# hellojialee/Improved-Body-Parts

Measured on NVIDIA H100. Metric: grouping images/sec @128x128 heatmaps, 30 persons/img, higher is better.
Workload: dtype f32 body-part maps, f32 keypoint maps; f64 coordinates/scores

## Files before the change

### improved_body_parts_b200/csrc/common.cuh

```cuda
#pragma once

#include <cuda_runtime.h>
#include <stdint.h>

#include <algorithm>

namespace spg {

#ifdef SPG_TRACE
constexpr int kTraceCtas = 64, kTraceSlots = 1024;
__device__ unsigned long long g_spg_trace[kTraceCtas * kTraceSlots];
__device__ __forceinline__ void trace_put(int slot, int dep, int mode) {
    if (blockIdx.x < kTraceCtas && (threadIdx.x & 31) == 0) {
        unsigned long long t;
        asm volatile("mov.u64 %0, %%clock64;" : "=l"(t) : "r"(dep) : "memory");
        unsigned long long *w = &g_spg_trace[blockIdx.x * kTraceSlots + slot];
        if (mode == 2) atomicCAS(w, 0ull, t);
        else if (mode == 3) atomicMax(w, t);
        else *w = mode == 1 ? (unsigned long long)(unsigned)dep : t;
    }
}
#define SPG_TR(slot, dep) ::spg::trace_put((slot), (int)(dep), 0)
#define SPG_TRV(slot, v) ::spg::trace_put((slot), (int)(v), 1)
#define SPG_TR_FIRST(slot, dep) ::spg::trace_put((slot), (int)(dep), 2)
#define SPG_TR_LAST(slot, dep) ::spg::trace_put((slot), (int)(dep), 3)
#else
#define SPG_TR(slot, dep) do {} while (0)
#define SPG_TRV(slot, v) do {} while (0)
#define SPG_TR_FIRST(slot, dep) do {} while (0)
#define SPG_TR_LAST(slot, dep) do {} while (0)
#endif

constexpr int kMaxParts = 32;
constexpr int kMaxLimbs = 64;
constexpr int kMaxCapPeaks = 128;
constexpr int kMaxCapRows = 128;
constexpr int kMaxRefineRadius = 4;
constexpr int kMaxOutJoints = 32;

constexpr uint32_t kStPeakOverflow = 1u << 0;
constexpr uint32_t kStCandOverflow = 1u << 1;
constexpr uint32_t kStRowOverflow = 1u << 2;
constexpr uint32_t kStSampleIndex = 1u << 3;
constexpr uint32_t kStAssert = 1u << 4;
constexpr uint32_t kStWireOverflow = 1u << 5;

struct Params {
    double thre1, thre2, connect_ration, len_rate, connection_tole, min_mean_score;
    int32_t mid_num, offset_radius, remove_recon, min_parts;
    int32_t crit1_strict, refresh_len_check;
};

struct Workspace {
    int K, L, J, capP, capC, capR, max_batch;
    int16_t limbs[kMaxLimbs * 2];
    int16_t out_from_part[kMaxOutJoints];
    double *peak_x, *peak_y;
    float *peak_score;
    uint32_t *peak_anchor;
    int32_t *peak_count;
    double *cand_prio, *cand_score;
    uint32_t *cand_ij;
    unsigned long long *cand_key;
    int32_t *cand_count;
    int32_t *surv_count;
    uint32_t *conn_ij;
    double *conn_score, *conn_norm;
    int32_t *conn_count;
    double *subset;
    int32_t *n_persons;
    double *people_xy;
    double *people_score;
    uint32_t *status;
    unsigned char *wire;
    long long wire_first;
    int wire_rows;
};

__device__ __forceinline__ uint32_t smem_u32(const void *p) { return (uint32_t)__cvta_generic_to_shared(p); }

__device__ __forceinline__ void mbar_init(uint64_t *bar, uint32_t count) {
    asm volatile("mbarrier.init.shared::cta.b64 [%0], %1;" ::"r"(smem_u32(bar)), "r"(count) : "memory");
}
__device__ __forceinline__ void fence_mbar_init() { asm volatile("fence.mbarrier_init.release.cluster;" ::: "memory"); }
__device__ __forceinline__ void fence_proxy_async() { asm volatile("fence.proxy.async.shared::cta;" ::: "memory"); }
__device__ __forceinline__ void mbar_expect_tx(uint64_t *bar, uint32_t bytes) {
    asm volatile("mbarrier.arrive.expect_tx.shared::cta.b64 _, [%0], %1;" ::"r"(smem_u32(bar)), "r"(bytes) : "memory");
}
__device__ __forceinline__ void bulk_g2s(void *dst_smem, const void *src_gmem, uint32_t bytes, uint64_t *bar) {
    asm volatile("cp.async.bulk.shared::cluster.global.mbarrier::complete_tx::bytes [%0], [%1], %2, [%3];" ::"r"(
                     smem_u32(dst_smem)),
                 "l"(src_gmem), "r"(bytes), "r"(smem_u32(bar))
                 : "memory");
}
__device__ __forceinline__ void mbar_arrive(uint64_t *bar) {
    asm volatile("mbarrier.arrive.shared::cta.b64 _, [%0];" ::"r"(smem_u32(bar)) : "memory");
}
__device__ __forceinline__ bool mbar_try_wait(uint64_t *bar, uint32_t parity) {
    uint32_t ok;
    asm volatile(
        "{\n"
        " .reg .pred p;\n"
        " mbarrier.try_wait.parity.shared::cta.b64 p, [%1], %2;\n"
        " selp.u32 %0, 1, 0, p;\n"
        "}\n"
        : "=r"(ok)
        : "r"(smem_u32(bar)), "r"(parity)
        : "memory");
    return ok != 0;
}
__device__ __forceinline__ void mbar_wait(uint64_t *bar, uint32_t parity) {
    while (!mbar_try_wait(bar, parity)) {
    }
}
__device__ __forceinline__ void mbar_wait_sleep(uint64_t *bar, uint32_t parity, uint32_t hint_ns = 20000u) {
    uint32_t ok = 0;
    while (!ok) {
        asm volatile(
            "{\n"
            " .reg .pred p;\n"
            " mbarrier.try_wait.parity.shared::cta.b64 p, [%1], %2, %3;\n"
            " selp.u32 %0, 1, 0, p;\n"
            "}\n"
            : "=r"(ok)
            : "r"(smem_u32(bar)), "r"(parity), "r"(hint_ns)
            : "memory");
    }
}

template <typename T>
__device__ __forceinline__ T pairwise_sum(const T *a, int n) {
    if (n < 8) {
        T res = (T)0;
        for (int i = 0; i < n; i++) res = res + a[i];
        return res;
    }
    T r[8];
#pragma unroll
    for (int k = 0; k < 8; k++) r[k] = a[k];
    int i = 8;
    for (; i < n - (n % 8); i += 8) {
#pragma unroll
        for (int k = 0; k < 8; k++) r[k] = r[k] + a[i + k];
    }
    T res = ((r[0] + r[1]) + (r[2] + r[3])) + ((r[4] + r[5]) + (r[6] + r[7]));
    for (; i < n; i++) res = res + a[i];
    return res;
}

}
```

### improved_body_parts_b200/csrc/nms_peaks.cuh

```cuda
#pragma once

#include "common.cuh"

namespace spg {

struct NmsArgs {
    const float *heat;
    int64_t img_stride, chan_stride;
    int H, W, band_rows, radius, use_bulk, image_base;
    float thr;
    Workspace ws;
};

constexpr int kNmsThreads = 256;
constexpr int kNmsBufs = 3;

__device__ __forceinline__ bool nms_is_peak(const float *buf, int lo, int H, int W, int y, int x, float v, float thr) {
    if (!(v >= thr) || v == 0.0f) return false;
#pragma unroll
    for (int dy = -1; dy <= 1; dy++) {
        const int yy = y + dy;
        if (yy < 0 || yy >= H) continue;
        const float *row = buf + (size_t)(yy - lo) * W;
#pragma unroll
        for (int dx = -1; dx <= 1; dx++) {
            const int xx = x + dx;
            if (xx < 0 || xx >= W) continue;
            if (!(row[xx] <= v)) return false;
        }
    }
    return true;
}

template <int R>
__device__ __forceinline__ void refine_box(const float *__restrict__ plane, int W, int x, int y, double &rx, double &ry,
                                           float &sc) {
    constexpr int D = 2 * R + 1, N = D * D;
    if (N == 1) {
        const float b = plane[(size_t)y * W + x];
        const float s32 = 0.0f + b;
        rx = __dadd_rn((double)x, __ddiv_rn(__dmul_rn((double)b, 0.0), (double)s32));
        ry = __dadd_rn((double)y, __ddiv_rn(__dmul_rn((double)b, 0.0), (double)s32));
        sc = __fdiv_rn(s32, 1.0f);
        return;
    }
    float s[8];
    double ax[8], ay[8];
    float ts = 0.0f;
    double tx = 0.0, ty = 0.0;
#pragma unroll
    for (int i = 0; i < N; i++) {
        const int r = i / D - R, q = i % D - R;
        const float b = plane[(size_t)(y + r) * W + (x + q)];
        const double wr = __dmul_rn((double)b, (double)r), wc = __dmul_rn((double)b, (double)q);
        if (i < 8) {
            s[i] = b; ax[i] = wr; ay[i] = wc;
        } else if (i < N - 1) {
            s[i & 7] = __fadd_rn(s[i & 7], b);
            ax[i & 7] = __dadd_rn(ax[i & 7], wr);
            ay[i & 7] = __dadd_rn(ay[i & 7], wc);
        } else {
            ts = b; tx = wr; ty = wc;
        }
    }
    const float s32 = __fadd_rn(__fadd_rn(__fadd_rn(__fadd_rn(s[0], s[1]), __fadd_rn(s[2], s[3])),
                                          __fadd_rn(__fadd_rn(s[4], s[5]), __fadd_rn(s[6], s[7]))), ts);
    const double sx = __dadd_rn(__dadd_rn(__dadd_rn(__dadd_rn(ax[0], ax[1]), __dadd_rn(ax[2], ax[3])),
                                          __dadd_rn(__dadd_rn(ax[4], ax[5]), __dadd_rn(ax[6], ax[7]))), tx);
    const double sy = __dadd_rn(__dadd_rn(__dadd_rn(__dadd_rn(ay[0], ay[1]), __dadd_rn(ay[2], ay[3])),
                                          __dadd_rn(__dadd_rn(ay[4], ay[5]), __dadd_rn(ay[6], ay[7]))), ty);
    rx = __dadd_rn((double)x, __ddiv_rn(sx, (double)s32));
    ry = __dadd_rn((double)y, __ddiv_rn(sy, (double)s32));
    sc = __fdiv_rn(s32, (float)N);
}

__device__ __forceinline__ void nms_test_group(const float *rows, int y, int x0, int H, int W, float thr, int *cnt, uint32_t *list, int capP) {
    const float *rc = rows + (size_t)y * W;
    const float *ru = rows + (size_t)max(y - 1, 0) * W;
    const float *rd = rows + (size_t)min(y + 1, H - 1) * W;
    const float4 c4 = *reinterpret_cast<const float4 *>(rc + x0);
    const float4 u4 = *reinterpret_cast<const float4 *>(ru + x0);
    const float4 d4 = *reinterpret_cast<const float4 *>(rd + x0);
    const int xl = max(x0 - 1, 0), xr = min(x0 + 4, W - 1);
    const float U[6] = {ru[xl], u4.x, u4.y, u4.z, u4.w, ru[xr]};
    const float C[6] = {rc[xl], c4.x, c4.y, c4.z, c4.w, rc[xr]};
    const float D[6] = {rd[xl], d4.x, d4.y, d4.z, d4.w, rd[xr]};
#pragma unroll
    for (int e = 0; e < 4; e++) {
        const float v = C[e + 1];
        const bool pk = (v >= thr) & (v != 0.0f) & (U[e] <= v) & (U[e + 1] <= v) & (U[e + 2] <= v) &
                        (C[e] <= v) & (C[e + 2] <= v) & (D[e] <= v) & (D[e + 1] <= v) & (D[e + 2] <= v);
        if (pk) {
            const int pos = atomicAdd(cnt, 1);
            if (pos < capP) list[pos] = (uint32_t)(y * W + x0 + e);
        }
    }
}

__device__ __forceinline__ void nms_finish_peak(const NmsArgs &a, const float *plane, int H, int W, size_t out, int lin) {
    const Workspace &ws = a.ws;
    const int R = a.radius;
    const int y = lin / W, x = lin - y * W;
    double rx, ry;
    float sc;
    uint32_t anchor = ((uint32_t)y << 16) | (uint32_t)x;
    if (y + R + 1 > H || y - R < 0 || x + R + 1 > W || x - R < 0) {
        rx = (double)x;
        ry = (double)y;
        sc = plane[(size_t)y * W + x];
        anchor |= 0x80000000u;
    } else {
        switch (R) {
            case 0: refine_box<0>(plane, W, x, y, rx, ry, sc); break;
            case 1: refine_box<1>(plane, W, x, y, rx, ry, sc); break;
            case 2: refine_box<2>(plane, W, x, y, rx, ry, sc); break;
            case 3: refine_box<3>(plane, W, x, y, rx, ry, sc); break;
            default: refine_box<4>(plane, W, x, y, rx, ry, sc); break;
        }
    }
    ws.peak_x[out] = rx;
    ws.peak_y[out] = ry;
    ws.peak_score[out] = sc;
    ws.peak_anchor[out] = anchor;
}

__device__ __forceinline__ void nms_publish_count(const NmsArgs &a, int n, int c, int total) {
    a.ws.peak_count[(size_t)n * a.ws.K + c] = total;
    if (total > a.ws.capP) atomicOr(&a.ws.status[n], kStPeakOverflow);
}

constexpr int kNmsPThreads = 1024;
constexpr int kNmsPFinishers = 3;
constexpr int kNmsPLists = 2 * kNmsPFinishers;
constexpr int kNmsPScanners = kNmsPThreads / 32 - 1 - kNmsPFinishers;
constexpr int kNmsPMaxIter = 5;

template <int ITER>
__device__ __forceinline__ int nms_queue_groups(const float *data, int g0, int g_step, int g_end, float thr, int lane, uint16_t *wq) {
    uint32_t am[ITER];
#pragma unroll
    for (int it = 0; it < ITER; it++) {
        const int g = g0 + it * g_step + lane;
        bool act = false;
        if (g < g_end) {
            const float4 c4 = *reinterpret_cast<const float4 *>(data + 4 * (size_t)g);
            act = fmaxf(fmaxf(c4.x, c4.y), fmaxf(c4.z, c4.w)) >= thr;
        }
        am[it] = __ballot_sync(0xffffffffu, act);
    }
    int nq = 0;
#pragma unroll
    for (int it = 0; it < ITER; it++) {
        const uint32_t m = am[it];
        if (m) {
            if ((m >> lane) & 1u) wq[nq + __popc(m & ((1u << lane) - 1u))] = (uint16_t)(g0 + it * g_step + lane);
            nq += __popc(m);
        }
    }
    __syncwarp();
    return nq;
}

__device__ __forceinline__ void nms_finish_plane(const NmsArgs &a, const uint32_t *list, int total, int item, int lane) {
    const int K = a.ws.K, capP = a.ws.capP;
    const int n_local = item / K, c = item - n_local * K;
    const float *plane = a.heat + (int64_t)n_local * a.img_stride + (int64_t)c * a.chan_stride;
    const int np = min(total, capP);
    const size_t out_base = ((size_t)(a.image_base + n_local) * K + c) * capP;
    for (int t = lane; t < np; t += 32) {
        const uint32_t mine = list[t];
        int rank = 0;
        for (int u = 0; u < np; u++) rank += list[u] < mine;
        nms_finish_peak(a, plane, a.H, a.W, out_base + rank, (int)mine);
    }
    if (lane == 0) nms_publish_count(a, a.image_base + n_local, c, total);
}

__global__ void __launch_bounds__(kNmsThreads, 4) nms_peaks_kernel(NmsArgs a) {
    extern __shared__ __align__(128) unsigned char smem_raw[];
    __shared__ uint64_t bar[kNmsBufs];
    __shared__ int s_count;

    const Workspace &ws = a.ws;
    const int tid = threadIdx.x;
    const int c = blockIdx.x % ws.K;
    const int n_local = blockIdx.x / ws.K;
    const int n = a.image_base + n_local;
    const int H = a.H, W = a.W, br = a.band_rows;
    const float *plane = a.heat + (int64_t)n_local * a.img_stride + (int64_t)c * a.chan_stride;

    const int nb = (H + br - 1) / br;
    const size_t band_floats = nb == 1 ? (size_t)H * W : (size_t)(br + 2) * W;
    const size_t buf_stride = (band_floats + 31) & ~(size_t)31;
    const int nbufs = min(nb, kNmsBufs);
    float *buf0 = reinterpret_cast<float *>(smem_raw);
    uint32_t *s_list = reinterpret_cast<uint32_t *>(buf0 + (size_t)nbufs * buf_stride);
    uint32_t *s_sorted = s_list + ws.capP;
    uint16_t *s_queue = reinterpret_cast<uint16_t *>(s_sorted + ws.capP);

    if (tid == 0) {
        s_count = 0;
        if (a.use_bulk) {
            for (int i = 0; i < kNmsBufs; i++) mbar_init(&bar[i], 1);
            fence_mbar_init();
        }
    }
    __syncthreads();

    auto band_lo = [&](int b) { return max(b * br - 1, 0); };
    auto band_hi = [&](int b) { return min((b + 1) * br + 1, H); };
    auto issue = [&](int b) {
        const int lo = band_lo(b), hi = band_hi(b);
        const uint32_t bytes = (uint32_t)(hi - lo) * W * sizeof(float);
        mbar_expect_tx(&bar[b % kNmsBufs], bytes);
        bulk_g2s(buf0 + (size_t)(b % kNmsBufs) * buf_stride, plane + (size_t)lo * W, bytes, &bar[b % kNmsBufs]);
    };

    if (a.use_bulk && tid == 0)
        for (int b = 0; b < nbufs; b++) issue(b);

    for (int b = 0; b < nb; b++) {
        float *buf = a.use_bulk ? buf0 + (size_t)(b % kNmsBufs) * buf_stride : buf0;
        const int lo = band_lo(b), hi = band_hi(b);
        if (a.use_bulk) {
            mbar_wait(&bar[b % kNmsBufs], (b / kNmsBufs) & 1);
        } else {
            const int cnt = (hi - lo) * W;
            for (int i = tid; i < cnt; i += kNmsThreads) buf[i] = plane[(size_t)lo * W + i];
            __syncthreads();
        }
        const int y0 = b * br, y1 = min(y0 + br, H);
        if ((W & 3) == 0) {
            const int W4 = W >> 2;
            const int groups = (y1 - y0) * W4;
            const int lane = tid & 31, warp = tid >> 5;
            const int gpw = (groups + (kNmsThreads / 32) - 1) / (kNmsThreads / 32);
            const int g_lo = warp * gpw, g_hi = min(g_lo + gpw, groups);
            uint16_t *wq = s_queue + g_lo;
            int nq = 0;
            for (int g0 = g_lo; g0 < g_hi; g0 += 32) {
                const int g = g0 + lane;
                bool act = false;
                if (g < g_hi) {
                    const float4 c4 = *reinterpret_cast<const float4 *>(buf + (size_t)(y0 - lo) * W + 4 * (size_t)g);
                    act = fmaxf(fmaxf(c4.x, c4.y), fmaxf(c4.z, c4.w)) >= a.thr;
                }
                const uint32_t am = __ballot_sync(0xffffffffu, act);
                if (act) wq[nq + __popc(am & ((1u << lane) - 1u))] = (uint16_t)g;
                nq += __popc(am);
            }
            __syncwarp();
            const float *rows = buf - (size_t)lo * W;
            for (int q = lane; q < nq; q += 32) {
                const int g = wq[q];
                const int r = g / W4, xq = g - r * W4;
                nms_test_group(rows, y0 + r, 4 * xq, H, W, a.thr, &s_count, s_list, ws.capP);
            }
        } else {
            const int cnt = (y1 - y0) * W;
            for (int i = tid; i < cnt; i += kNmsThreads) {
                const int r = i / W, x = i - r * W;
                const int y = y0 + r;
                const float v = buf[(size_t)(y - lo) * W + x];
                if (nms_is_peak(buf, lo, H, W, y, x, v, a.thr)) {
                    const int pos = atomicAdd(&s_count, 1);
                    if (pos < ws.capP) s_list[pos] = (uint32_t)(y * W + x);
                }
            }
        }
        __syncthreads();
        if (a.use_bulk && tid == 0 && b + kNmsBufs < nb) issue(b + kNmsBufs);
    }

    const int total = s_count;
    const int np = min(total, ws.capP);
    for (int t = tid; t < np; t += kNmsThreads) {
        const uint32_t mine = s_list[t];
        int rank = 0;
        for (int u = 0; u < np; u++) rank += s_list[u] < mine;
        s_sorted[rank] = mine;
    }
    __syncthreads();
    const size_t out_base = ((size_t)n * ws.K + c) * ws.capP;
    for (int t = tid; t < np; t += kNmsThreads) nms_finish_peak(a, plane, H, W, out_base + t, (int)s_sorted[t]);
    if (tid == 0) nms_publish_count(a, n, c, total);
}

inline size_t nms_smem_bytes(int band_rows, int H, int W, int capP) {
    const bool single = band_rows >= H;
    const size_t band_floats = ((single ? (size_t)H * W : (size_t)(band_rows + 2) * W) + 31) & ~(size_t)31;
    const size_t queue = (((size_t)std::min(band_rows, H) * W / 4 + 8) * sizeof(uint16_t) + 15) & ~(size_t)15;
    const int nb = single ? 1 : (H + band_rows - 1) / band_rows;
    return (size_t)std::min(nb, kNmsBufs) * band_floats * sizeof(float) + 2 * (size_t)capP * sizeof(uint32_t) + queue;
}

}
```

### improved_body_parts_b200/csrc/nms_peaks_banded.cuh

```cuda
#pragma once

#include "nms_peaks_persist.cuh"

namespace spg {

constexpr int kNmsBMaxSlots = 16;
constexpr int kNmsBTeams = 4;
constexpr int kNmsBBandGroups = 1024;

struct NmsBanding {
    int band_rows, n_bands, slots, teams;
    size_t band_stride, smem;
};
inline NmsBanding nms_banding(int H, int W, int capP, size_t smem_limit) {
    NmsBanding g{};
    const int W4 = W / 4;
    const size_t fixed = kNmsPLists * (size_t)capP * sizeof(uint32_t) + (size_t)kNmsPScanners * 32 * kNmsPMaxIter * sizeof(uint16_t) + 64;
    if (smem_limit <= fixed) return g;
    g.teams = kNmsBTeams;
    const int team_warps = kNmsPScanners / kNmsBTeams;
    g.band_rows = std::max(1, std::min(H, kNmsBBandGroups / std::max(W4, 1)));
    if ((size_t)g.band_rows * W4 > (size_t)team_warps * 32 * kNmsPMaxIter) return g;
    g.n_bands = (H + g.band_rows - 1) / g.band_rows;
    g.band_stride = (((size_t)std::min(g.band_rows + 2, H) * W * sizeof(float)) + 127) & ~(size_t)127;
    g.slots = (int)std::min<size_t>(kNmsBMaxSlots, (smem_limit - fixed) / g.band_stride) / kNmsBTeams * kNmsBTeams;
    g.smem = (size_t)g.slots * g.band_stride + fixed;
    return g;
}

__global__ void __launch_bounds__(kNmsPThreads, 1) nms_peaks_banded_kernel(NmsArgs a, int n_items, int n_slots, int n_bands) {
    extern __shared__ __align__(128) unsigned char smem_raw[];
    __shared__ uint64_t bar_full[kNmsBMaxSlots], bar_free[kNmsBMaxSlots], bar_ready[kNmsPLists], bar_lfree[kNmsPLists];
    __shared__ int s_cnt[kNmsPLists];

    const Workspace &ws = a.ws;
    const int tid = threadIdx.x, lane = tid & 31, warp = tid >> 5;
    const int H = a.H, W = a.W, K = ws.K, capP = ws.capP;
    const int BR = a.band_rows, S = n_slots, NB = n_bands;
    constexpr int T = kNmsBTeams, TW = kNmsPScanners / kNmsBTeams;
    const size_t band_stride = (((size_t)min(BR + 2, H) * W * sizeof(float)) + 127) & ~(size_t)127;
    uint32_t *s_lists = reinterpret_cast<uint32_t *>(smem_raw + (size_t)S * band_stride);
    uint16_t *s_queues = reinterpret_cast<uint16_t *>(s_lists + kNmsPLists * (size_t)capP);
    const int W4 = W >> 2;
    const uint32_t w4_magic = W4 > 1 ? 0xffffffffu / (uint32_t)W4 + 1u : 0u;

    if (tid == 0) {
        for (int s = 0; s < S; s++) {
            mbar_init(&bar_full[s], 1);
            mbar_init(&bar_free[s], TW);
        }
        for (int l = 0; l < kNmsPLists; l++) {
            mbar_init(&bar_ready[l], kNmsPScanners);
            mbar_init(&bar_lfree[l], 1);
            s_cnt[l] = 0;
        }
        fence_mbar_init();
    }
    __syncthreads();

    const int G = gridDim.x;
    const int nj = ((int)blockIdx.x < n_items) ? (n_items - 1 - (int)blockIdx.x) / G + 1 : 0;

    if (warp == 0) {
        if (lane == 0) {
            int s = 0, round = 0;
            for (int j = 0; j < nj; j++) {
                const int item = (int)blockIdx.x + j * G;
                const int n_local = item / K, c = item - n_local * K;
                const float *plane = a.heat + (int64_t)n_local * a.img_stride + (int64_t)c * a.chan_stride;
                for (int b = 0; b < NB; b++) {
                    if (round > 0) mbar_wait_sleep(&bar_free[s], (round - 1) & 1);
                    const int r0 = b * BR, lo = max(r0 - 1, 0), hi = min(r0 + BR + 1, H);
                    const uint32_t bytes = (uint32_t)((size_t)(hi - lo) * W * sizeof(float));
                    mbar_expect_tx(&bar_full[s], bytes);
                    bulk_g2s(smem_raw + (size_t)s * band_stride, plane + (size_t)lo * W, bytes, &bar_full[s]);
                    if (++s == S) { s = 0; round++; }
                }
            }
        }
    } else if (warp <= kNmsPScanners) {
        const int w = warp - 1, team = w / TW, tw = w - team * TW;
        uint16_t *wq = s_queues + (size_t)w * (32 * kNmsPMaxIter);
        const float thr = a.thr;
        for (int j = 0; j < nj; j++) {
            const int l = j % kNmsPLists;
            uint32_t *list = s_lists + (size_t)l * capP;
            if (j >= kNmsPLists) mbar_wait_sleep(&bar_lfree[l], ((j / kNmsPLists) - 1) & 1);
            for (int b = (team - (j * NB) % T + T) % T; b < NB; b += T) {
                const int t = j * NB + b, round = t / S, s = t - round * S;
                mbar_wait_sleep(&bar_full[s], round & 1);
                const int r0 = b * BR, r1 = min(r0 + BR, H), lo = max(r0 - 1, 0);
                const int groups = (r1 - r0) * W4;
                const float *band = reinterpret_cast<const float *>(smem_raw + (size_t)s * band_stride) - (size_t)lo * W;
                const int nq = nms_queue_groups<kNmsPMaxIter>(band + (size_t)r0 * W, tw * 32, TW * 32, groups, thr, lane, wq);
                for (int q = lane; q < nq; q += 32) {
                    const int g = wq[q];
                    const int yl = W4 > 1 ? (int)__umulhi((uint32_t)g, w4_magic) : g, xq = g - yl * W4;
                    const int y = r0 + yl, x0 = 4 * xq;
                    nms_test_group(band, y, x0, H, W, thr, &s_cnt[l], list, capP);
                }
                __syncwarp();
                if (lane == 0) mbar_arrive(&bar_free[s]);
            }
            __syncwarp();
            if (lane == 0) mbar_arrive(&bar_ready[l]);
        }
    } else {
        const int f = warp - 1 - kNmsPScanners;
        for (int j = f; j < nj; j += kNmsPFinishers) {
            const int l = j % kNmsPLists;
            mbar_wait_sleep(&bar_ready[l], (j / kNmsPLists) & 1);
            nms_finish_plane(a, s_lists + (size_t)l * capP, s_cnt[l], (int)blockIdx.x + j * G, lane);
            __syncwarp();
            if (lane == 0) {
                s_cnt[l] = 0;
                mbar_arrive(&bar_lfree[l]);
            }
        }
    }
}

}
```

### improved_body_parts_b200/csrc/nms_peaks_persist.cuh

```cuda
#pragma once

#include "nms_peaks.cuh"

namespace spg {

constexpr int kNmsPSlots = 3;

inline size_t nms_persist_smem_bytes(int H, int W, int capP) {
    const size_t plane = (((size_t)H * W * sizeof(float)) + 127) & ~(size_t)127;
    const size_t gpw = ((size_t)H * W / 4 + kNmsPScanners - 1) / kNmsPScanners;
    const size_t queues = ((gpw * kNmsPScanners * sizeof(uint16_t)) + 15) & ~(size_t)15;
    return kNmsPSlots * plane + kNmsPLists * (size_t)capP * sizeof(uint32_t) + queues + 64;
}

__global__ void __launch_bounds__(kNmsPThreads, 1) nms_peaks_persist_kernel(NmsArgs a, int n_items) {
    extern __shared__ __align__(128) unsigned char smem_raw[];
    __shared__ uint64_t bar_full[kNmsPSlots], bar_free[kNmsPSlots], bar_ready[kNmsPLists], bar_lfree[kNmsPLists];
    __shared__ int s_cnt[kNmsPLists];

    const Workspace &ws = a.ws;
    const int tid = threadIdx.x, lane = tid & 31, warp = tid >> 5;
    const int H = a.H, W = a.W, K = ws.K, capP = ws.capP;
    const size_t plane_bytes = (size_t)H * W * sizeof(float);
    const size_t plane_stride = (plane_bytes + 127) & ~(size_t)127;
    uint32_t *s_lists = reinterpret_cast<uint32_t *>(smem_raw + kNmsPSlots * plane_stride);
    uint16_t *s_queues = reinterpret_cast<uint16_t *>(s_lists + kNmsPLists * (size_t)capP);
    const int W4 = W >> 2, groups = H * W4;
    const uint32_t w4_magic = W4 > 1 ? 0xffffffffu / (uint32_t)W4 + 1u : 0u;
    const int gpw = (groups + kNmsPScanners - 1) / kNmsPScanners;

    if (tid == 0) {
        for (int s = 0; s < kNmsPSlots; s++) {
            mbar_init(&bar_full[s], 1);
            mbar_init(&bar_free[s], kNmsPScanners);
        }
        for (int l = 0; l < kNmsPLists; l++) {
            mbar_init(&bar_ready[l], kNmsPScanners);
            mbar_init(&bar_lfree[l], 1);
            s_cnt[l] = 0;
        }
        fence_mbar_init();
    }
    __syncthreads();

    const int G = gridDim.x;
    const int nj = ((int)blockIdx.x < n_items) ? (n_items - 1 - (int)blockIdx.x) / G + 1 : 0;

    if (warp == 0) {
        if (lane == 0) {
            for (int j = 0; j < nj; j++) {
                const int s = j % kNmsPSlots;
                if (j >= kNmsPSlots) mbar_wait_sleep(&bar_free[s], ((j / kNmsPSlots) - 1) & 1);
                const int item = (int)blockIdx.x + j * G;
                const int n_local = item / K, c = item - n_local * K;
                const unsigned char *src =
                    reinterpret_cast<const unsigned char *>(a.heat + (int64_t)n_local * a.img_stride + (int64_t)c * a.chan_stride);
                unsigned char *dst = smem_raw + s * plane_stride;
                mbar_expect_tx(&bar_full[s], (uint32_t)plane_bytes);
                for (size_t off = 0; off < plane_bytes; off += 32768) {
                    const uint32_t bytes = (uint32_t)min((size_t)32768, plane_bytes - off);
                    bulk_g2s(dst + off, src + off, bytes, &bar_full[s]);
                }
            }
        }
    } else if (warp <= kNmsPScanners) {
        const int w = warp - 1;
        uint16_t *wq = s_queues + (size_t)w * gpw;
        const int g_lo = w * gpw, g_hi = min(g_lo + gpw, groups);
        const float thr = a.thr;
        for (int j = 0; j < nj; j++) {
            const int s = j % kNmsPSlots, l = j % kNmsPLists;
            mbar_wait_sleep(&bar_full[s], (j / kNmsPSlots) & 1);
            if (j >= kNmsPLists) mbar_wait_sleep(&bar_lfree[l], ((j / kNmsPLists) - 1) & 1);
            const float *buf = reinterpret_cast<const float *>(smem_raw + s * plane_stride);
            uint32_t *list = s_lists + (size_t)l * capP;
            const int nq = nms_queue_groups<kNmsPMaxIter>(buf, g_lo, 32, g_hi, thr, lane, wq);
            for (int q = lane; q < nq; q += 32) {
                const int g = wq[q];
                const int y = W4 > 1 ? (int)__umulhi((uint32_t)g, w4_magic) : g, xq = g - y * W4;
                nms_test_group(buf, y, 4 * xq, H, W, thr, &s_cnt[l], list, capP);
            }
            __syncwarp();
            if (lane == 0) {
                mbar_arrive(&bar_free[s]);
                mbar_arrive(&bar_ready[l]);
            }
        }
    } else {
        const int f = warp - 1 - kNmsPScanners;
        for (int j = f; j < nj; j += kNmsPFinishers) {
            const int l = j % kNmsPLists;
            mbar_wait_sleep(&bar_ready[l], (j / kNmsPLists) & 1);
            nms_finish_plane(a, s_lists + (size_t)l * capP, s_cnt[l], (int)blockIdx.x + j * G, lane);
            __syncwarp();
            if (lane == 0) {
                s_cnt[l] = 0;
                mbar_arrive(&bar_lfree[l]);
            }
        }
    }
}

}
```

### improved_body_parts_b200/csrc/spgroup.cu

```cuda
#include "../../include/spgroup.h"

#include <cuda_runtime.h>

#include <algorithm>
#include <cstdarg>
#include <cstdio>
#include <cstdlib>
#include <cstring>
#include <new>
#include <string>
#include <vector>

#include "assemble.cuh"
#include "common.cuh"
#include "limb_match.cuh"
#include "limb_score.cuh"
#include "limb_score_persist.cuh"
#include "match_assemble.cuh"
#include "nms_peaks.cuh"
#include "nms_peaks_persist.cuh"
#include "nms_peaks_banded.cuh"
#include "postnet.cuh"

using namespace spg;

static_assert(sizeof(spg_params) == sizeof(spg::Params), "spg_params layout");

static thread_local std::string g_create_error;

struct spg_handle {
    spg_config cfg{};
    int device = 0;
    int sm_count = 0;
    size_t smem_optin = 0;
    Workspace ws{};
    std::vector<void *> allocs;
    void *in_heat = nullptr, *in_paf = nullptr;
    size_t in_heat_bytes = 0, in_paf_bytes = 0;
    unsigned int *done_counter = nullptr;
    unsigned long long *armed_flag = nullptr;
    unsigned long long armed_value = 0;
    double *heat_acc = nullptr;
    size_t heat_acc_elems = 0;
    cudaStream_t streams[2] = {nullptr, nullptr};
    int64_t launches = 0;
    const char *stage_kernel[5] = {"", "", "", "", ""};
    int persist = 1;
    int screen = 1;
    int exact_warps = 14;
    int ma_warps = kMAMatchWarps;
    int fuse_ma = 1;
    int cand_dtype = SPG_F32;
    int stage = 0;
    std::string err;
};

namespace {

int fail(spg_handle *h, int code, const char *fmt, ...) {
    char buf[512];
    va_list ap;
    va_start(ap, fmt);
    vsnprintf(buf, sizeof buf, fmt, ap);
    va_end(ap);
    if (h) h->err = buf; else g_create_error = buf;
    return code;
}

#define SPG_CUDA(h, call)                                                                              \
    do {                                                                                               \
        cudaError_t e_ = (call);                                                                       \
        if (e_ != cudaSuccess) return fail((h), SPG_E_CUDA, "%s failed: %s", #call, cudaGetErrorString(e_)); \
    } while (0)

template <typename T>
int dalloc(spg_handle *h, T **p, size_t count) {
    void *q = nullptr;
    SPG_CUDA(h, cudaMalloc(&q, std::max<size_t>(count, 1) * sizeof(T)));
    h->allocs.push_back(q);
    *p = static_cast<T *>(q);
    return SPG_OK;
}

struct DeviceGuard {
    int prev = -1;
    explicit DeviceGuard(int dev) {
        cudaGetDevice(&prev);
        if (prev != dev) cudaSetDevice(dev);
    }
    ~DeviceGuard() {
        int cur = -1;
        cudaGetDevice(&cur);
        if (prev >= 0 && cur != prev) cudaSetDevice(prev);
    }
};

int check_dims(spg_handle *h, int n, int H, int W) {
    if (n < 0 || n > h->cfg.max_batch) return fail(h, SPG_E_INVALID, "n_images %d outside [0, max_batch=%d]", n, h->cfg.max_batch);
    if (H < 2 || W < 2 || H > h->cfg.max_h || W > h->cfg.max_w || H > 32767 || W > 32767)
        return fail(h, SPG_E_INVALID, "map %dx%d outside [2, %dx%d]", H, W, h->cfg.max_h, h->cfg.max_w);
    return SPG_OK;
}

int check_params(spg_handle *h, const spg_params *p) {
    if (!p) return fail(h, SPG_E_INVALID, "params is NULL");
    if (p->offset_radius < 0 || p->offset_radius > kMaxRefineRadius)
        return fail(h, SPG_E_INVALID, "offset_radius %d outside [0, %d]", p->offset_radius, kMaxRefineRadius);
    if (p->mid_num < 1) return fail(h, SPG_E_INVALID, "mid_num must be >= 1");
    return SPG_OK;
}

int launch_nms(spg_handle *h, const float *heat, int64_t img_stride, int64_t chan_stride, int base, int n, int H, int W,
               const spg_params *p, cudaStream_t st) {
    if (n == 0) return SPG_OK;
    NmsArgs a{};
    a.heat = heat;
    a.img_stride = img_stride;
    a.chan_stride = chan_stride;
    a.H = H;
    a.W = W;
    a.radius = p->offset_radius;
    a.use_bulk = (W % 4 == 0) && (img_stride % 4 == 0) && (chan_stride % 4 == 0) && ((reinterpret_cast<uintptr_t>(heat) & 15) == 0);
    a.image_base = base;
    a.thr = (float)p->thre1;
    a.ws = h->ws;
    if (h->persist && a.use_bulk && nms_persist_smem_bytes(H, W, h->ws.capP) <= h->smem_optin && (size_t)H * W / 4 < 65536 &&
        (size_t)H * W * sizeof(float) < (1u << 20) &&
        ((size_t)H * W / 4 + kNmsPScanners - 1) / kNmsPScanners <= (size_t)32 * kNmsPMaxIter) {
        const size_t psm = nms_persist_smem_bytes(H, W, h->ws.capP);
        const int items = n * h->ws.K;
        SPG_CUDA(h, cudaFuncSetAttribute(nms_peaks_persist_kernel, cudaFuncAttributeMaxDynamicSharedMemorySize, (int)psm));
        nms_peaks_persist_kernel<<<std::min(items, h->sm_count), kNmsPThreads, psm, st>>>(a, items);
        h->stage_kernel[0] = "nms_peaks_persist_kernel";
        h->launches++;
        SPG_CUDA(h, cudaGetLastError());
        return SPG_OK;
    }
    const NmsBanding bg = (h->persist && a.use_bulk) ? nms_banding(H, W, h->ws.capP, h->smem_optin - 1024) : NmsBanding{};
    if (bg.slots >= kNmsBTeams) {
        const int items = n * h->ws.K;
        a.band_rows = bg.band_rows;
        SPG_CUDA(h, cudaFuncSetAttribute(nms_peaks_banded_kernel, cudaFuncAttributeMaxDynamicSharedMemorySize, (int)bg.smem));
        nms_peaks_banded_kernel<<<std::min(items, h->sm_count), kNmsPThreads, bg.smem, st>>>(a, items, bg.slots, bg.n_bands);
        h->stage_kernel[0] = "nms_peaks_banded_kernel";
        h->launches++;
        SPG_CUDA(h, cudaGetLastError());
        return SPG_OK;
    }
    a.band_rows = std::max(4, std::min(H, 4096 / W));
    const size_t smem = nms_smem_bytes(a.band_rows, H, W, h->ws.capP);
    if (smem > h->smem_optin) return fail(h, SPG_E_INVALID, "map width %d needs %zu B of shared memory per band", W, smem);
    SPG_CUDA(h, cudaFuncSetAttribute(nms_peaks_kernel, cudaFuncAttributeMaxDynamicSharedMemorySize, (int)smem));
    nms_peaks_kernel<<<n * h->ws.K, kNmsThreads, smem, st>>>(a);
    h->stage_kernel[0] = "nms_peaks_kernel";
    h->launches++;
    SPG_CUDA(h, cudaGetLastError());
    return SPG_OK;
}

template <typename T, typename TA = T>
int launch_score_t(spg_handle *h, const ScoreArgs &a, int n, cudaStream_t st) {
    const size_t plane_bytes = (size_t)a.H * a.W * sizeof(T);
    const size_t staged = score_smem_bytes(plane_bytes, h->ws.capP);
    const bool aligned = (plane_bytes % 16 == 0) && ((a.img_stride * sizeof(T)) % 16 == 0) && ((a.chan_stride * sizeof(T)) % 16 == 0) &&
                         ((reinterpret_cast<uintptr_t>(a.paf) & 15) == 0) && plane_bytes < (1u << 20);
    const int grid = n * h->ws.L;
    if (sizeof(T) == 4 && h->persist && aligned && h->ws.capP <= kPersistMaxCapP &&
        persist_smem_bytes(plane_bytes, h->ws.capP) <= h->smem_optin) {
        const size_t smem = persist_smem_bytes(plane_bytes, h->ws.capP);
        SPG_CUDA(h, cudaFuncSetAttribute(limb_score_persist_kernel<TA>, cudaFuncAttributeMaxDynamicSharedMemorySize, (int)smem));
        limb_score_persist_kernel<TA><<<std::min(grid, h->sm_count), kPersistThreads, smem, st>>>(a, grid);
        h->stage_kernel[1] = sizeof(TA) == 4 ? "limb_score_persist_kernel<float>" : "limb_score_persist_kernel<double>";
    } else if (aligned && staged <= h->smem_optin) {
        SPG_CUDA(h, (cudaFuncSetAttribute(limb_score_kernel<T, true, TA>, cudaFuncAttributeMaxDynamicSharedMemorySize, (int)staged)));
        limb_score_kernel<T, true, TA><<<grid, kScoreThreads, staged, st>>>(a);
        h->stage_kernel[1] = sizeof(T) == 8 ? "limb_score_kernel<double,true>" : sizeof(TA) == 4 ? "limb_score_kernel<float,true>" : "limb_score_kernel<float,true,double>";
    } else {
        const size_t smem = score_smem_bytes(0, h->ws.capP);
        limb_score_kernel<T, false, TA><<<grid, kScoreThreads, smem, st>>>(a);
        h->stage_kernel[1] = sizeof(T) == 8 ? "limb_score_kernel<double,false>" : sizeof(TA) == 4 ? "limb_score_kernel<float,false>" : "limb_score_kernel<float,false,double>";
    }
    h->launches++;
    SPG_CUDA(h, cudaGetLastError());
    return SPG_OK;
}

int launch_score(spg_handle *h, const void *paf, int dtype, int64_t img_stride, int64_t chan_stride, int base, int n, int H,
                 int W, double extent, const spg_params *p, cudaStream_t st) {
    if (n == 0) return SPG_OK;
    ScoreArgs a{};
    a.paf = paf;
    a.img_stride = img_stride;
    a.chan_stride = chan_stride;
    a.H = H;
    a.W = W;
    a.image_base = base;
    a.mid_num = p->mid_num;
    a.image_extent = extent;
    a.thre2 = p->thre2;
    a.connect_ration = p->connect_ration;
    a.screen = h->screen;
    a.crit1_strict = p->crit1_strict != 0;
    a.exact_warps = h->exact_warps;
    a.ws = h->ws;
    h->cand_dtype = dtype;
    if (dtype == SPG_F64) return launch_score_t<double>(h, a, n, st);
    if (dtype == SPG_F32_AS_F64) return launch_score_t<float, double>(h, a, n, st);
    return launch_score_t<float>(h, a, n, st);
}

int launch_match(spg_handle *h, int base, int n, cudaStream_t st) {
    if (n == 0) return SPG_OK;
    MatchArgs a{};
    a.n_images = n;
    a.image_base = base;
    a.keys_valid = h->cand_dtype == SPG_F32;
    a.ws = h->ws;
    const int warps = n * h->ws.L;
    const int blocks = (warps * 32 + kMatchThreads - 1) / kMatchThreads;
    limb_match_kernel<<<blocks, kMatchThreads, 0, st>>>(a);
    h->stage_kernel[2] = "limb_match_kernel";
    h->launches++;
    SPG_CUDA(h, cudaGetLastError());
    return SPG_OK;
}

AssembleArgs assemble_args(const spg_handle *h, int base, int n, const spg_params *p) {
    AssembleArgs a{};
    a.n_images = n;
    a.image_base = base;
    a.len_rate = p->len_rate;
    a.connection_tole = p->connection_tole;
    a.min_mean_score = p->min_mean_score;
    a.remove_recon = p->remove_recon;
    a.min_parts = p->min_parts;
    a.refresh_len_check = p->refresh_len_check != 0;
    a.wire_flag = h->armed_flag; a.wire_flag_value = h->armed_value; a.done_counter = h->done_counter;
    a.ws = h->ws;
    a.ws.wire_first += base;
    return a;
}

int launch_assemble(spg_handle *h, int base, int n, const spg_params *p, cudaStream_t st) {
    if (n == 0) return SPG_OK;
    AssembleArgs a = assemble_args(h, base, n, p);
    h->armed_flag = nullptr;
    a.use_bulk = ((size_t)h->ws.L * h->ws.capP * sizeof(uint32_t)) % 16 == 0;
    const size_t smem = assemble_smem_bytes(h->ws.K, h->ws.capP, h->ws.capR) + assemble_conn_bytes(h->ws.L, h->ws.capP);
    if (smem > h->smem_optin) return fail(h, SPG_E_INVALID, "capacities need %zu B of shared memory in assemble (limit %zu)", smem, h->smem_optin);
    SPG_CUDA(h, cudaFuncSetAttribute(assemble_kernel, cudaFuncAttributeMaxDynamicSharedMemorySize, (int)smem));
    assemble_kernel<<<n, kAssembleThreads, smem, st>>>(a);
    h->stage_kernel[3] = "assemble_kernel";
    h->launches++;
    SPG_CUDA(h, cudaGetLastError());
    return SPG_OK;
}

int launch_match_assemble(spg_handle *h, int base, int n, const spg_params *p, cudaStream_t st) {
    if (n == 0) return SPG_OK;
    AssembleArgs a = assemble_args(h, base, n, p);
    a.use_bulk = ((size_t)h->ws.K * h->ws.capP * sizeof(float)) % 16 == 0;
    const size_t smem = match_assemble_smem_bytes(h->ws.K, h->ws.L, h->ws.capP, h->ws.capR, h->ma_warps);
    if (smem > h->smem_optin) {
        int rc;
        if ((rc = launch_match(h, base, n, st))) return rc;
        return launch_assemble(h, base, n, p, st);
    }
    h->armed_flag = nullptr;
    SPG_CUDA(h, cudaFuncSetAttribute(match_assemble_kernel, cudaFuncAttributeMaxDynamicSharedMemorySize, (int)smem));
    match_assemble_kernel<<<n, 32 * (1 + h->ma_warps), smem, st>>>(a, h->cand_dtype == SPG_F32);
    h->stage_kernel[2] = "match_assemble_kernel";
    h->stage_kernel[3] = "";
    h->launches++;
    SPG_CUDA(h, cudaGetLastError());
    return SPG_OK;
}

int run_all(spg_handle *h, const float *heat, int64_t his, int64_t hcs, const void *paf, int dtype, int64_t pis, int64_t pcs,
            int base, int n, int H, int W, double extent, const spg_params *p, cudaStream_t st) {
    int rc;
    SPG_CUDA(h, cudaMemsetAsync(h->ws.status + base, 0, sizeof(uint32_t) * (size_t)n, st));
    if ((rc = launch_nms(h, heat, his, hcs, base, n, H, W, p, st))) return rc;
    if ((rc = launch_score(h, paf, dtype, pis, pcs, base, n, H, W, extent, p, st))) return rc;
    if (h->fuse_ma) return launch_match_assemble(h, base, n, p, st);
    if ((rc = launch_match(h, base, n, st))) return rc;
    if ((rc = launch_assemble(h, base, n, p, st))) return rc;
    return SPG_OK;
}

__global__ void wire_signal_kernel(unsigned long long *word, unsigned long long value) {
    __threadfence_system();
    asm volatile("st.release.sys.global.u64 [%0], %1;" ::"l"(word), "l"(value) : "memory");
}

struct WireWords {
    unsigned long long *p[32];
    int n;
};
__global__ void wire_signal_many_kernel(WireWords w, unsigned long long value) {
    __threadfence_system();
    if ((int)threadIdx.x < w.n) asm volatile("st.release.sys.global.u64 [%0], %1;" ::"l"(w.p[threadIdx.x]), "l"(value) : "memory");
}

__global__ void wire_wait_kernel(const unsigned long long *word, unsigned long long value) {
    unsigned long long v;
    do {
        asm volatile("ld.acquire.sys.global.u64 %0, [%1];" : "=l"(v) : "l"(word) : "memory");
        if (v < value) __nanosleep(500);
    } while (v < value);
}

}

extern "C" {

#ifdef SPG_TRACE
int spg_trace_read(unsigned long long *out, size_t n_words, int clear) {
    const size_t n = std::min(n_words, (size_t)spg::kTraceCtas * spg::kTraceSlots);
    if (cudaMemcpyFromSymbol(out, spg::g_spg_trace, n * sizeof(unsigned long long)) != cudaSuccess) return -1;
    if (clear) {
        void *p = nullptr;
        if (cudaGetSymbolAddress(&p, spg::g_spg_trace) != cudaSuccess) return -1;
        if (cudaMemset(p, 0, sizeof(spg::g_spg_trace)) != cudaSuccess) return -1;
    }
    return 0;
}
#endif

int spg_abi_version(void) { return SPG_ABI_VERSION; }

const char *spg_last_error(const spg_handle *h) { return h ? h->err.c_str() : g_create_error.c_str(); }

int spg_create(const spg_config *cfg, spg_handle **out) {
    if (!cfg || !out) return fail(nullptr, SPG_E_INVALID, "cfg/out is NULL");
    *out = nullptr;
    if (cfg->abi_version != SPG_ABI_VERSION) return fail(nullptr, SPG_E_INVALID, "ABI version %d != %d", cfg->abi_version, SPG_ABI_VERSION);
    if (cfg->n_parts < 1 || cfg->n_parts > kMaxParts || cfg->n_limbs < 1 || cfg->n_limbs > kMaxLimbs || !cfg->limbs)
        return fail(nullptr, SPG_E_INVALID, "n_parts in [1,%d], n_limbs in [1,%d], limbs non-NULL required", kMaxParts, kMaxLimbs);
    if (cfg->n_out_joints < 0 || cfg->n_out_joints > kMaxOutJoints || (cfg->n_out_joints && !cfg->out_from_part))
        return fail(nullptr, SPG_E_INVALID, "n_out_joints in [0,%d]", kMaxOutJoints);
    if (cfg->max_peaks_per_part < 1 || cfg->max_peaks_per_part > kMaxCapPeaks)
        return fail(nullptr, SPG_E_INVALID, "max_peaks_per_part in [1,%d]", kMaxCapPeaks);
    if (cfg->max_person_rows < 1 || cfg->max_person_rows > kMaxCapRows)
        return fail(nullptr, SPG_E_INVALID, "max_person_rows in [1,%d]", kMaxCapRows);
    if (cfg->max_cands_per_limb < 1 || cfg->max_batch < 1 || cfg->max_h < 2 || cfg->max_w < 2)
        return fail(nullptr, SPG_E_INVALID, "max_cands_per_limb, max_batch >= 1 and max_h, max_w >= 2 required");
    for (int k = 0; k < cfg->n_limbs * 2; k++)
        if (cfg->limbs[k] < 0 || cfg->limbs[k] >= cfg->n_parts) return fail(nullptr, SPG_E_INVALID, "limb table entry %d out of range", k);
    for (int g = 0; g < cfg->n_out_joints; g++)
        if (cfg->out_from_part[g] < 0 || cfg->out_from_part[g] >= cfg->n_parts) return fail(nullptr, SPG_E_INVALID, "out_from_part[%d] out of range", g);

    int ndev = 0;
    if (cudaGetDeviceCount(&ndev) != cudaSuccess || ndev == 0) return fail(nullptr, SPG_E_NO_DEVICE, "no CUDA device (this library has no CPU path)");
    if (cfg->device < 0 || cfg->device >= ndev) return fail(nullptr, SPG_E_INVALID, "device %d outside [0,%d)", cfg->device, ndev);
    cudaDeviceProp prop{};
    if (cudaGetDeviceProperties(&prop, cfg->device) != cudaSuccess) return fail(nullptr, SPG_E_CUDA, "cudaGetDeviceProperties failed");
    if (prop.major != 9 || prop.minor != 0) return fail(nullptr, SPG_E_NO_DEVICE, "device %d is sm_%d%d; this library is built for sm_90a only", cfg->device, prop.major, prop.minor);

    spg_handle *h = new (std::nothrow) spg_handle();
    if (!h) return fail(nullptr, SPG_E_INVALID, "out of host memory");
    h->cfg = *cfg;
    h->cfg.limbs = nullptr;
    h->cfg.out_from_part = nullptr;
    h->device = cfg->device;
    h->sm_count = prop.multiProcessorCount;
    h->smem_optin = prop.sharedMemPerBlockOptin;
    if (const char *e = getenv("SPG_NO_SCREEN")) h->screen = !(e[0] == '1');
    if (const char *e = getenv("SPG_PERSIST")) h->persist = !(e[0] == '0');
    if (const char *e = getenv("SPG_MA_WARPS")) h->ma_warps = std::max(1, std::min(15, atoi(e)));
    if (const char *e = getenv("SPG_FUSE_MA")) h->fuse_ma = !(e[0] == '0');
    if (const char *e = getenv("SPG_EXACT_WARPS")) h->exact_warps = std::max(1, std::min(30, atoi(e)));
    DeviceGuard guard(h->device);

    const size_t N = cfg->max_batch, K = cfg->n_parts, L = cfg->n_limbs, J = cfg->n_out_joints;
    const size_t cP = cfg->max_peaks_per_part, cC = cfg->max_cands_per_limb, cR = cfg->max_person_rows;
    Workspace &ws = h->ws;
    ws.K = (int)K; ws.L = (int)L; ws.J = (int)J; ws.capP = (int)cP; ws.capC = (int)cC; ws.capR = (int)cR; ws.max_batch = (int)N;
    int rc = SPG_OK;
    auto A = [&](int r) { if (rc == SPG_OK) rc = r; };
    A(dalloc(h, &ws.peak_x, N * K * cP));
    A(dalloc(h, &ws.peak_y, N * K * cP));
    A(dalloc(h, &ws.peak_score, N * K * cP));
    A(dalloc(h, &ws.peak_anchor, N * K * cP));
    A(dalloc(h, &ws.peak_count, N * K));
    A(dalloc(h, &ws.cand_prio, N * L * cC));
    A(dalloc(h, &ws.cand_score, N * L * cC));
    A(dalloc(h, &ws.cand_ij, N * L * cC));
    A(dalloc(h, &ws.cand_key, N * L * cC));
    A(dalloc(h, &ws.cand_count, N * L));
    A(dalloc(h, &ws.surv_count, N * L));
    A(dalloc(h, &ws.conn_ij, N * L * cP));
    A(dalloc(h, &ws.conn_score, N * L * cP));
    A(dalloc(h, &ws.conn_norm, N * L * cP));
    A(dalloc(h, &ws.conn_count, N * L));
    A(dalloc(h, &ws.subset, N * cR * (K + 2) * 2));
    A(dalloc(h, &ws.n_persons, N));
    A(dalloc(h, &ws.people_xy, N * cR * std::max<size_t>(J, 1) * 2));
    A(dalloc(h, &ws.people_score, N * cR));
    A(dalloc(h, &ws.status, N));
    for (size_t i = 0; i < L * 2; i++) ws.limbs[i] = (int16_t)cfg->limbs[i];
    for (size_t g = 0; g < J; g++) ws.out_from_part[g] = (int16_t)cfg->out_from_part[g];
    if (rc == SPG_OK && cudaMemset(ws.status, 0, sizeof(uint32_t) * N) != cudaSuccess) rc = SPG_E_CUDA;
    if (rc == SPG_OK && cudaMemset(ws.peak_count, 0, sizeof(int32_t) * N * K) != cudaSuccess) rc = SPG_E_CUDA;
    for (int s = 0; s < 2 && rc == SPG_OK; s++)
        if (cudaStreamCreateWithFlags(&h->streams[s], cudaStreamNonBlocking) != cudaSuccess) rc = SPG_E_CUDA;
    if (rc != SPG_OK) {
        g_create_error = h->err.empty() ? "device allocation failed" : h->err;
        spg_destroy(h);
        return rc;
    }
    *out = h;
    return SPG_OK;
}

void spg_destroy(spg_handle *h) {
    if (!h) return;
    DeviceGuard guard(h->device);
    cudaDeviceSynchronize();
    for (void *p : h->allocs) cudaFree(p);
    if (h->in_heat) cudaFree(h->in_heat);
    if (h->in_paf) cudaFree(h->in_paf);
    if (h->heat_acc) cudaFree(h->heat_acc);
    if (h->done_counter) cudaFree(h->done_counter);
    for (auto &s : h->streams)
        if (s) cudaStreamDestroy(s);
    delete h;
}

int spg_get_device_view(const spg_handle *h, spg_device_view *v) {
    if (!h || !v) return SPG_E_INVALID;
    const Workspace &ws = h->ws;
    v->max_batch = ws.max_batch; v->n_parts = ws.K; v->n_limbs = ws.L; v->n_out_joints = ws.J;
    v->cap_peaks = ws.capP; v->cap_cands = ws.capC; v->cap_rows = ws.capR;
    v->peak_x = ws.peak_x; v->peak_y = ws.peak_y; v->peak_score = ws.peak_score; v->peak_anchor = ws.peak_anchor;
    v->peak_count = ws.peak_count;
// ... 532 lines not shown
```

Before: 590,500.

## Refine peaks from staged smem plane and interleave NMS scanner work

The persistent NMS kernel now runs sub-pixel refinement on the plane already staged in shared memory instead of re-reading global memory. To support this, the staging slot is released by the finisher warp rather than by the scanners. Scanners now take 32-group chunks in a strided pattern, and they wait for the list-free barrier only after queueing candidates. The refine radius becomes a template parameter, and coordinates are decoded with a magic-multiply instead of a division. The trade-off is that each staging slot stays occupied longer, which may stall the producer, and the change adds several kernel instantiations and trace hooks.

```diff
diff --git a/improved_body_parts_b200/csrc/common.cuh b/improved_body_parts_b200/csrc/common.cuh
--- a/improved_body_parts_b200/csrc/common.cuh
+++ b/improved_body_parts_b200/csrc/common.cuh
@@ -17,6 +17,7 @@
         unsigned long long *w = &g_spg_trace[blockIdx.x * kTraceSlots + slot];
         if (mode == 2) atomicCAS(w, 0ull, t);
         else if (mode == 3) atomicMax(w, t);
+        else if (mode == 4) atomicAdd(w, (unsigned long long)(unsigned)dep);
         else *w = mode == 1 ? (unsigned long long)(unsigned)dep : t;
     }
 }
@@ -24,11 +25,13 @@
 #define SPG_TRV(slot, v) ::spg::trace_put((slot), (int)(v), 1)
 #define SPG_TR_FIRST(slot, dep) ::spg::trace_put((slot), (int)(dep), 2)
 #define SPG_TR_LAST(slot, dep) ::spg::trace_put((slot), (int)(dep), 3)
+#define SPG_TR_ADD(slot, v) ::spg::trace_put((slot), (int)(v), 4)
 #else
 #define SPG_TR(slot, dep) do {} while (0)
 #define SPG_TRV(slot, v) do {} while (0)
 #define SPG_TR_FIRST(slot, dep) do {} while (0)
 #define SPG_TR_LAST(slot, dep) do {} while (0)
+#define SPG_TR_ADD(slot, v) do {} while (0)
 #endif
 
 constexpr int kMaxParts = 32;
diff --git a/improved_body_parts_b200/csrc/nms_peaks.cuh b/improved_body_parts_b200/csrc/nms_peaks.cuh
--- a/improved_body_parts_b200/csrc/nms_peaks.cuh
+++ b/improved_body_parts_b200/csrc/nms_peaks.cuh
@@ -97,20 +97,22 @@
     }
 }
 
-__device__ __forceinline__ void nms_finish_peak(const NmsArgs &a, const float *plane, int H, int W, size_t out, int lin) {
+template <int R = -1>
+__device__ __forceinline__ void nms_finish_peak(const NmsArgs &a, const float *plane, int H, int W, size_t out, int y, int x) {
     const Workspace &ws = a.ws;
-    const int R = a.radius;
-    const int y = lin / W, x = lin - y * W;
+    const int r = R >= 0 ? R : a.radius;
     double rx, ry;
     float sc;
     uint32_t anchor = ((uint32_t)y << 16) | (uint32_t)x;
-    if (y + R + 1 > H || y - R < 0 || x + R + 1 > W || x - R < 0) {
+    if (y + r + 1 > H || y - r < 0 || x + r + 1 > W || x - r < 0) {
         rx = (double)x;
         ry = (double)y;
         sc = plane[(size_t)y * W + x];
         anchor |= 0x80000000u;
+    } else if constexpr (R >= 0) {
+        refine_box<R>(plane, W, x, y, rx, ry, sc);
     } else {
-        switch (R) {
+        switch (r) {
             case 0: refine_box<0>(plane, W, x, y, rx, ry, sc); break;
             case 1: refine_box<1>(plane, W, x, y, rx, ry, sc); break;
             case 2: refine_box<2>(plane, W, x, y, rx, ry, sc); break;
@@ -161,17 +163,20 @@
     return nq;
 }
 
-__device__ __forceinline__ void nms_finish_plane(const NmsArgs &a, const uint32_t *list, int total, int item, int lane) {
-    const int K = a.ws.K, capP = a.ws.capP;
+template <int R = -1>
+__device__ __forceinline__ void nms_finish_plane(const NmsArgs &a, const uint32_t *list, int total, int item, int lane,
+                                                 uint32_t w4_magic, const float *staged = nullptr) {
+    const int K = a.ws.K, capP = a.ws.capP, W = a.W;
     const int n_local = item / K, c = item - n_local * K;
-    const float *plane = a.heat + (int64_t)n_local * a.img_stride + (int64_t)c * a.chan_stride;
+    const float *plane = staged ? staged : a.heat + (int64_t)n_local * a.img_stride + (int64_t)c * a.chan_stride;
     const int np = min(total, capP);
     const size_t out_base = ((size_t)(a.image_base + n_local) * K + c) * capP;
     for (int t = lane; t < np; t += 32) {
         const uint32_t mine = list[t];
         int rank = 0;
         for (int u = 0; u < np; u++) rank += list[u] < mine;
-        nms_finish_peak(a, plane, a.H, a.W, out_base + rank, (int)mine);
+        const int y = w4_magic ? (int)__umulhi(mine >> 2, w4_magic) : (int)mine / W, x = (int)mine - y * W;
+        nms_finish_peak<R>(a, plane, a.H, W, out_base + rank, y, x);
     }
     if (lane == 0) nms_publish_count(a, a.image_base + n_local, c, total);
 }
@@ -282,7 +287,10 @@
     }
     __syncthreads();
     const size_t out_base = ((size_t)n * ws.K + c) * ws.capP;
-    for (int t = tid; t < np; t += kNmsThreads) nms_finish_peak(a, plane, H, W, out_base + t, (int)s_sorted[t]);
+    for (int t = tid; t < np; t += kNmsThreads) {
+        const int lin = (int)s_sorted[t], y = lin / W;
+        nms_finish_peak(a, plane, H, W, out_base + t, y, lin - y * W);
+    }
     if (tid == 0) nms_publish_count(a, n, c, total);
 }
 
diff --git a/improved_body_parts_b200/csrc/nms_peaks_banded.cuh b/improved_body_parts_b200/csrc/nms_peaks_banded.cuh
--- a/improved_body_parts_b200/csrc/nms_peaks_banded.cuh
+++ b/improved_body_parts_b200/csrc/nms_peaks_banded.cuh
@@ -110,7 +110,7 @@
         for (int j = f; j < nj; j += kNmsPFinishers) {
             const int l = j % kNmsPLists;
             mbar_wait_sleep(&bar_ready[l], (j / kNmsPLists) & 1);
-            nms_finish_plane(a, s_lists + (size_t)l * capP, s_cnt[l], (int)blockIdx.x + j * G, lane);
+            nms_finish_plane(a, s_lists + (size_t)l * capP, s_cnt[l], (int)blockIdx.x + j * G, lane, 0u);
             __syncwarp();
             if (lane == 0) {
                 s_cnt[l] = 0;
diff --git a/improved_body_parts_b200/csrc/nms_peaks_persist.cuh b/improved_body_parts_b200/csrc/nms_peaks_persist.cuh
--- a/improved_body_parts_b200/csrc/nms_peaks_persist.cuh
+++ b/improved_body_parts_b200/csrc/nms_peaks_persist.cuh
@@ -6,13 +6,16 @@
 
 constexpr int kNmsPSlots = 3;
 
+constexpr int kNmsTrWords = 16, kNmsTrPlanes = 64;
+#define SPG_NMS_TR(kind, j, f, dep) do { if ((j) < kNmsTrPlanes) kind(kNmsTrWords * (j) + (f), dep); } while (0)
+
 inline size_t nms_persist_smem_bytes(int H, int W, int capP) {
     const size_t plane = (((size_t)H * W * sizeof(float)) + 127) & ~(size_t)127;
-    const size_t gpw = ((size_t)H * W / 4 + kNmsPScanners - 1) / kNmsPScanners;
-    const size_t queues = ((gpw * kNmsPScanners * sizeof(uint16_t)) + 15) & ~(size_t)15;
+    const size_t queues = (size_t)kNmsPScanners * 32 * kNmsPMaxIter * sizeof(uint16_t);
     return kNmsPSlots * plane + kNmsPLists * (size_t)capP * sizeof(uint32_t) + queues + 64;
 }
 
+template <int R>
 __global__ void __launch_bounds__(kNmsPThreads, 1) nms_peaks_persist_kernel(NmsArgs a, int n_items) {
     extern __shared__ __align__(128) unsigned char smem_raw[];
     __shared__ uint64_t bar_full[kNmsPSlots], bar_free[kNmsPSlots], bar_ready[kNmsPLists], bar_lfree[kNmsPLists];
@@ -27,12 +30,11 @@
     uint16_t *s_queues = reinterpret_cast<uint16_t *>(s_lists + kNmsPLists * (size_t)capP);
     const int W4 = W >> 2, groups = H * W4;
     const uint32_t w4_magic = W4 > 1 ? 0xffffffffu / (uint32_t)W4 + 1u : 0u;
-    const int gpw = (groups + kNmsPScanners - 1) / kNmsPScanners;
 
     if (tid == 0) {
         for (int s = 0; s < kNmsPSlots; s++) {
             mbar_init(&bar_full[s], 1);
-            mbar_init(&bar_free[s], kNmsPScanners);
+            mbar_init(&bar_free[s], 1);
         }
         for (int l = 0; l < kNmsPLists; l++) {
             mbar_init(&bar_ready[l], kNmsPScanners);
@@ -50,6 +52,7 @@
         if (lane == 0) {
             for (int j = 0; j < nj; j++) {
                 const int s = j % kNmsPSlots;
+                SPG_NMS_TR(SPG_TR, j, 0, j);
                 if (j >= kNmsPSlots) mbar_wait_sleep(&bar_free[s], ((j / kNmsPSlots) - 1) & 1);
                 const int item = (int)blockIdx.x + j * G;
                 const int n_local = item / K, c = item - n_local * K;
@@ -61,20 +64,24 @@
                     const uint32_t bytes = (uint32_t)min((size_t)32768, plane_bytes - off);
                     bulk_g2s(dst + off, src + off, bytes, &bar_full[s]);
                 }
+                SPG_NMS_TR(SPG_TR, j, 1, j);
             }
         }
     } else if (warp <= kNmsPScanners) {
         const int w = warp - 1;
-        uint16_t *wq = s_queues + (size_t)w * gpw;
-        const int g_lo = w * gpw, g_hi = min(g_lo + gpw, groups);
+        uint16_t *wq = s_queues + (size_t)w * (32 * kNmsPMaxIter);
         const float thr = a.thr;
         for (int j = 0; j < nj; j++) {
             const int s = j % kNmsPSlots, l = j % kNmsPLists;
             mbar_wait_sleep(&bar_full[s], (j / kNmsPSlots) & 1);
-            if (j >= kNmsPLists) mbar_wait_sleep(&bar_lfree[l], ((j / kNmsPLists) - 1) & 1);
+            SPG_NMS_TR(SPG_TR_FIRST, j, 2, j);
             const float *buf = reinterpret_cast<const float *>(smem_raw + s * plane_stride);
             uint32_t *list = s_lists + (size_t)l * capP;
-            const int nq = nms_queue_groups<kNmsPMaxIter>(buf, g_lo, 32, g_hi, thr, lane, wq);
+            const int nq = nms_queue_groups<kNmsPMaxIter>(buf, w * 32, kNmsPScanners * 32, groups, thr, lane, wq);
+            SPG_NMS_TR(SPG_TR_LAST, j, 5, nq);
+            SPG_NMS_TR(SPG_TR_ADD, j, 11, nq);
+            if (j >= kNmsPLists) mbar_wait_sleep(&bar_lfree[l], ((j / kNmsPLists) - 1) & 1);
+            SPG_NMS_TR(SPG_TR_LAST, j, 4, j);
             for (int q = lane; q < nq; q += 32) {
                 const int g = wq[q];
                 const int y = W4 > 1 ? (int)__umulhi((uint32_t)g, w4_magic) : g, xq = g - y * W4;
@@ -82,18 +89,27 @@
             }
             __syncwarp();
             if (lane == 0) {
-                mbar_arrive(&bar_free[s]);
+                SPG_NMS_TR(SPG_TR_FIRST, j, 6, j);
+                SPG_NMS_TR(SPG_TR_LAST, j, 7, j);
                 mbar_arrive(&bar_ready[l]);
+                SPG_NMS_TR(SPG_TR_LAST, j, 8, j);
             }
         }
     } else {
         const int f = warp - 1 - kNmsPScanners;
         for (int j = f; j < nj; j += kNmsPFinishers) {
             const int l = j % kNmsPLists;
+            SPG_NMS_TR(SPG_TR, j, 13, j);
             mbar_wait_sleep(&bar_ready[l], (j / kNmsPLists) & 1);
-            nms_finish_plane(a, s_lists + (size_t)l * capP, s_cnt[l], (int)blockIdx.x + j * G, lane);
+            SPG_NMS_TR(SPG_TR, j, 9, j);
+            SPG_NMS_TR(SPG_TRV, j, 12, s_cnt[l]);
+            const int s = j % kNmsPSlots;
+            nms_finish_plane<R>(a, s_lists + (size_t)l * capP, s_cnt[l], (int)blockIdx.x + j * G, lane, w4_magic,
+                                reinterpret_cast<const float *>(smem_raw + s * plane_stride));
             __syncwarp();
+            SPG_NMS_TR(SPG_TR, j, 10, j);
             if (lane == 0) {
+                mbar_arrive(&bar_free[s]);
                 s_cnt[l] = 0;
                 mbar_arrive(&bar_lfree[l]);
             }
diff --git a/improved_body_parts_b200/csrc/spgroup.cu b/improved_body_parts_b200/csrc/spgroup.cu
--- a/improved_body_parts_b200/csrc/spgroup.cu
+++ b/improved_body_parts_b200/csrc/spgroup.cu
@@ -129,8 +129,16 @@
         ((size_t)H * W / 4 + kNmsPScanners - 1) / kNmsPScanners <= (size_t)32 * kNmsPMaxIter) {
         const size_t psm = nms_persist_smem_bytes(H, W, h->ws.capP);
         const int items = n * h->ws.K;
-        SPG_CUDA(h, cudaFuncSetAttribute(nms_peaks_persist_kernel, cudaFuncAttributeMaxDynamicSharedMemorySize, (int)psm));
-        nms_peaks_persist_kernel<<<std::min(items, h->sm_count), kNmsPThreads, psm, st>>>(a, items);
+        void (*kern)(NmsArgs, int) = nms_peaks_persist_kernel<kMaxRefineRadius>;
+        switch (a.radius) {
+            case 0: kern = nms_peaks_persist_kernel<0>; break;
+            case 1: kern = nms_peaks_persist_kernel<1>; break;
+            case 2: kern = nms_peaks_persist_kernel<2>; break;
+            case 3: kern = nms_peaks_persist_kernel<3>; break;
+        }
+        static_assert(kMaxRefineRadius == 4, "one nms_peaks_persist_kernel instantiation per radius");
+        SPG_CUDA(h, cudaFuncSetAttribute(kern, cudaFuncAttributeMaxDynamicSharedMemorySize, (int)psm));
+        kern<<<std::min(items, h->sm_count), kNmsPThreads, psm, st>>>(a, items);
         h->stage_kernel[0] = "nms_peaks_persist_kernel";
         h->launches++;
         SPG_CUDA(h, cudaGetLastError());
```

After: 619,900, median of 6. 5.0% higher.
